# Mistra-UEA/Mistra

Hardware: AMD Instinct MI355X
Metric: chemistry-timesteps/sec (tot mechanism) (higher is better)
Workload: dtype f64; 1 GPU; tot mechanism, 100000 synthetic cells per GPU (100000 total), INTEGRATE_t(0,10 s), Ros3 rtol 1e-3; perturbed captured BTZ96 cloud states; cells_per_gpu=100000, failed_cells=0, parallelism=cells sharded over 1 GPU(s), no data-path collective

## Files before the change

mistra_amd/csrc/ros3_kernel.hip:

```cpp
#include <hip/hip_runtime.h>

#include <cstdint>
#include <type_traits>

#include "kernel_args.hpp"
#include "ros3_kernel.hpp"
#include "ros_methods.hpp"
#include "wave_ops.hpp"

namespace mistra {

namespace {

constexpr uint16_t kPosDiag = 0x8000, kPosNone = 0xFFFF;
constexpr int kRingSlots = 8;

#ifndef MISTRA_STREAM_GSUM_BARRIER
#define MISTRA_STREAM_GSUM_BARRIER 1
#endif
#ifndef MISTRA_STREAM_GSUM_CHAIN
#define MISTRA_STREAM_GSUM_CHAIN 1
#endif
#ifndef MISTRA_STREAM_SWEEP_BARRIER
#define MISTRA_STREAM_SWEEP_BARRIER 1
// ... 558 lines not shown
  const int n = __builtin_amdgcn_readfirstlane(P.nslots);
  gptr<u32x4> rp = G_(reinterpret_cast<const u32x4*>(P.recs)) + ((size_t)wave * (size_t)P.wave_slots * 64 + lane);
  asm volatile("s_waitcnt vmcnt(0)" : : : "memory");
  vm_ring_load<LOW, 0>(rp);       vm_ring_load<LOW, 1>(rp + 64);  vm_ring_load<LOW, 2>(rp + 128); vm_ring_load<LOW, 3>(rp + 192);
  vm_ring_load<LOW, 4>(rp + 256); vm_ring_load<LOW, 5>(rp + 320); vm_ring_load<LOW, 6>(rp + 384); vm_ring_load<LOW, 7>(rp + 448);
  rp += kRingSlots * 64;
  constexpr bool TRIM = MISTRA_STREAM_SCALE_TRIM && !LOW;
  const int n_refilled = TRIM ? n - kRingSlots : n;
#define MISTRA_SCALE_GROUP(K, REFILL)                                                \
    {                                                                                \
      const u32x4 a0 = vm_ring_take<LOW, K, REFILL ? 7 : 7 - K>();     if constexpr (REFILL) vm_ring_load<LOW, K>(rp + K * 64);         \
      const u32x4 a1 = vm_ring_take<LOW, K + 1, REFILL ? 7 : 6 - K>(); if constexpr (REFILL) vm_ring_load<LOW, K + 1>(rp + (K + 1) * 64); \
      const u32x4 a2 = vm_ring_take<LOW, K + 2, REFILL ? 7 : 5 - K>(); if constexpr (REFILL) vm_ring_load<LOW, K + 2>(rp + (K + 2) * 64); \
      const u32x4 a3 = vm_ring_take<LOW, K + 3, REFILL ? 7 : 4 - K>(); if constexpr (REFILL) vm_ring_load<LOW, K + 3>(rp + (K + 3) * 64); \
      const double v0 = lds_ld(a0.x), f0 = lds_ld(a0.y), v1 = lds_ld(a0.z), f1 = lds_ld(a0.w); \
      const double v2 = lds_ld(a1.x), f2 = lds_ld(a1.y), v3 = lds_ld(a1.z), f3 = lds_ld(a1.w); \
      const double v4 = lds_ld(a2.x), f4 = lds_ld(a2.y), v5 = lds_ld(a2.z), f5 = lds_ld(a2.w); \
      const double v6 = lds_ld(a3.x), f6 = lds_ld(a3.y), v7 = lds_ld(a3.z), f7 = lds_ld(a3.w); \
      lds_st(a0.x, v0 * f0); lds_st(a0.z, v1 * f1); lds_st(a1.x, v2 * f2); lds_st(a1.z, v3 * f3); \
      lds_st(a2.x, v4 * f4); lds_st(a2.z, v5 * f5); lds_st(a3.x, v6 * f6); lds_st(a3.z, v7 * f7); \
    }
  for (int i = 0; i < n_refilled; i += kRingSlots) {
    MISTRA_SCALE_GROUP(0, true) MISTRA_SCALE_GROUP(4, true)
    rp += kRingSlots * 64;
  }
  if constexpr (TRIM) {
    if (n > 0) { MISTRA_SCALE_GROUP(0, false) MISTRA_SCALE_GROUP(4, false) }
  }
#undef MISTRA_SCALE_GROUP
  asm volatile("s_waitcnt vmcnt(0)" : : : "memory");
}

#ifdef MISTRA_DIAG_STAMPS
__device__ unsigned long long g_dense_stamps[16];
#define MISTRA_STAMP(var) const unsigned long long var = clock64();
#define MISTRA_STAMP_ADD(slot, expr) if (threadIdx.x == 0) atomicAdd(&g_dense_stamps[slot], (unsigned long long)(expr));
#else
#define MISTRA_STAMP(var)
#define MISTRA_STAMP_ADD(slot, expr)
#endif
typedef double f64x4 __attribute__((ext_vector_type(4)));
typedef uint32_t u32x2 __attribute__((ext_vector_type(2)));
typedef __attribute__((address_space(3))) f64x4 lds_f64x4;
__device__ __forceinline__ f64x4 lds_ld4(uint32_t addr) { return *(const lds_f64x4*)(uintptr_t)addr; }
__device__ __forceinline__ void lds_st4(uint32_t addr, f64x4 v) { *(lds_f64x4*)(uintptr_t)addr = v; }
typedef __attribute__((address_space(3))) __attribute__((aligned(16))) f64x4 lds_f64x4_a16;
__device__ __forceinline__ f64x4 lds_ld4_a16(uint32_t addr) { return *(const lds_f64x4_a16*)(uintptr_t)addr; }
__device__ __forceinline__ void lds_st4_a16(uint32_t addr, f64x4 v) { *(lds_f64x4_a16*)(uintptr_t)addr = v; }

__device__ __forceinline__ uint32_t dense_slot(const u32x4 info, const uint32_t c, const uint32_t zero) {
  const uint64_t absent = (uint64_t)info.y | ((uint64_t)info.z << 32);
  const uint32_t idx = info.x + c - (uint32_t)__builtin_popcountll(absent & ((1ull << c) - 1ull));
  return ((absent >> c) & 1ull) ? zero : 8u * idx;
}
typedef __attribute__((address_space(3))) u32x4 lds_u32x4;
__device__ __forceinline__ u32x4 lds_ldu4(uint32_t addr) { return *(const lds_u32x4*)(uintptr_t)addr; }

__device__ __forceinline__ bool dense_is_storer(const int wave) { return wave == 1 || wave == 2 || wave == 3 || wave == 5; }
template <class MT, int NT>
__device__ __forceinline__ void dense_store_panel(const int P, const int wave, const int lane) {
  constexpr uint32_t NNZ = MT::NNZ, NVAR = MT::NVAR, H = NVAR - 64, ZERO = 8u * (NNZ + NVAR);
  constexpr uint32_t PB = 8u * (uint32_t)LdsLayout<MT, NT>::PANEL, BC = PB + 8192u, INFO = 8u * (uint32_t)LdsLayout<MT, NT>::DINFO;
  const uint32_t PL = PB + (uint32_t)(P & 1) * 4096u, PU = PL + 2048u;
  const int J0P = 4 * P, khalf = (wave == 3 || wave == 5) ? 2 : 0;
  const f64x4 rcp = lds_ld4(BC + 1024u + 32u * (uint32_t)(P & 1));
  if (wave & 1) {
    if (wave != 5) {
// ... 72 lines not shown
    a[2] = a[2] * rcp[2];
    a[3] = __builtin_fma(-a[2], d23, a[3]);
    a[3] = a[3] * rcp[3];
    b[1] = __builtin_fma(-l10, b[0], b[1]); b[2] = __builtin_fma(-l20, b[0], b[2]); b[3] = __builtin_fma(-l30, b[0], b[3]);
    b[2] = __builtin_fma(-l21, b[1], b[2]); b[3] = __builtin_fma(-l31, b[1], b[3]);
    b[3] = __builtin_fma(-l32, b[2], b[3]);
    lds_st4(PL + 32u * lane, a);
    lds_st4(PU + 32u * lane, b);
    if (lane == 0) lds_st4(BC + 1024u + 32u * (uint32_t)(P & 1), rcp);
  } else if (dense_is_storer(wave) && P > 0) {
    dense_store_panel<MT, NT>(P - 1, wave, lane);
  }
  MISTRA_STAMP(tc)
  lds_barrier();
  MISTRA_STAMP(td)
  if (I >= K2) {
    const double aop = (int)(16u * I + lcol) >= J0P + 4 ? -lds_ld(PL + 8u * ((16u * I + lcol) * 4u + lrow)) : 0.0;
    if (J0 >= K2) {
      const double bop = (int)(16u * J0 + lcol) >= J0P + 4 ? lds_ld(PU + 8u * ((16u * J0 + lcol) * 4u + lrow)) : 0.0;
      T0 = __builtin_amdgcn_mfma_f64_16x16x4f64(aop, bop, T0, 0, 0, 0);
    }
    if (J0 + 1 >= K2) {
      const double bop = (int)(16u * (J0 + 1) + lcol) >= J0P + 4 ? lds_ld(PU + 8u * ((16u * (J0 + 1) + lcol) * 4u + lrow)) : 0.0;
      T1 = __builtin_amdgcn_mfma_f64_16x16x4f64(aop, bop, T1, 0, 0, 0);
    }
  }
  MISTRA_STAMP(te)
#ifdef MISTRA_DIAG_STAMPS
  acc[0] += tb - ta; acc[1] += tc - tb; acc[2] += td - tc; acc[3] += te - td; acc[4] += 1;
#endif
}

#define MISTRA_FIN_F(J, C) "v_fmac_f64_dpp %[x" #C "], -%[x" #C "], %[l] row_newbcast:" #J " row_mask:0xf bank_mask:0xf\n\t"
#define MISTRA_FIN_FROM_15(J) MISTRA_FIN_F(J, 15)
#define MISTRA_FIN_FROM_14(J) MISTRA_FIN_F(J, 14) MISTRA_FIN_FROM_15(J)
#define MISTRA_FIN_FROM_13(J) MISTRA_FIN_F(J, 13) MISTRA_FIN_FROM_14(J)
#define MISTRA_FIN_FROM_12(J) MISTRA_FIN_F(J, 12) MISTRA_FIN_FROM_13(J)
#define MISTRA_FIN_FROM_11(J) MISTRA_FIN_F(J, 11) MISTRA_FIN_FROM_12(J)
#define MISTRA_FIN_FROM_10(J) MISTRA_FIN_F(J, 10) MISTRA_FIN_FROM_11(J)
#define MISTRA_FIN_FROM_9(J) MISTRA_FIN_F(J, 9) MISTRA_FIN_FROM_10(J)
#define MISTRA_FIN_FROM_8(J) MISTRA_FIN_F(J, 8) MISTRA_FIN_FROM_9(J)
#define MISTRA_FIN_FROM_7(J) MISTRA_FIN_F(J, 7) MISTRA_FIN_FROM_8(J)
#define MISTRA_FIN_FROM_6(J) MISTRA_FIN_F(J, 6) MISTRA_FIN_FROM_7(J)
#define MISTRA_FIN_FROM_5(J) MISTRA_FIN_F(J, 5) MISTRA_FIN_FROM_6(J)
#define MISTRA_FIN_FROM_4(J) MISTRA_FIN_F(J, 4) MISTRA_FIN_FROM_5(J)
#define MISTRA_FIN_FROM_3(J) MISTRA_FIN_F(J, 3) MISTRA_FIN_FROM_4(J)
#define MISTRA_FIN_FROM_2(J) MISTRA_FIN_F(J, 2) MISTRA_FIN_FROM_3(J)
#define MISTRA_FIN_FROM_1(J) MISTRA_FIN_F(J, 1) MISTRA_FIN_FROM_2(J)
#define MISTRA_FIN_XS [x0] "+v"(x0), [x1] "+v"(x1), [x2] "+v"(x2), [x3] "+v"(x3), [x4] "+v"(x4), [x5] "+v"(x5), [x6] "+v"(x6), [x7] "+v"(x7), \
                      [x8] "+v"(x8), [x9] "+v"(x9), [x10] "+v"(x10), [x11] "+v"(x11), [x12] "+v"(x12), [x13] "+v"(x13), [x14] "+v"(x14), [x15] "+v"(x15)
#define MISTRA_FIN_PIVOT(J, J1)                                                                                                       \
  {                                                                                                                                   \
    double dg, l;                                                                                                                     \
    asm volatile("s_nop 1\n\tv_mov_b64_dpp %[dg], %[x] row_newbcast:" #J " row_mask:0xf bank_mask:0xf" : [dg] "=v"(dg) : [x] "v"(x##J));       \
    const double R = 1.0 / dg;                                                                                                        \
    constexpr uint32_t GE = ((0xffffu << J) & 0xffffu) * 0x10001u, GT = ((0xffffu << J1) & 0xffffu) * 0x10001u;                       \
    asm volatile("v_mov_b64 %[l], %[nz]\n\t"                                                                                          \
                 "s_mov_b32 exec_lo, %[gt]\n\ts_mov_b32 exec_hi, %[gt]\n\t"                                                           \
                 "v_mul_f64 %[l], %[x" #J "], %[R]\n\t"                                                                               \
                 "v_mul_f64 %[x" #J "], %[x" #J "], %[R]\n\t"                                                                         \
                 "s_mov_b32 exec_lo, %[ge]\n\ts_mov_b32 exec_hi, %[ge]\n\t"                                                           \
                 MISTRA_FIN_FROM_##J1(J)                                                                                              \
                 "s_mov_b64 exec, -1"                                                                                                 \
                 : [l] "=&v"(l), MISTRA_FIN_XS : [R] "v"(R), [nz] "v"(nz), [gt] "i"((int)GT), [ge] "i"((int)GE));                               \
  }
template <class MT, int NT>
__device__ __attribute__((noinline)) void dense_finish(const f64x4 T, const int lane) {
  constexpr uint32_t NNZ = MT::NNZ, NVAR = MT::NVAR, H = NVAR - 64, ZERO = 8u * (NNZ + NVAR);
  constexpr uint32_t INFO = 8u * (uint32_t)LdsLayout<MT, NT>::DINFO, RDIAG = 8u * (NNZ + NVAR + 4u);
  constexpr uint32_t BUF = 8u * (uint32_t)LdsLayout<MT, NT>::PANEL, STRIDE = 144u;
  const uint32_t lrow = (uint32_t)(lane >> 4), i = (uint32_t)(lane & 15);
  MISTRA_STAMP(tf0)
#pragma unroll
  for (int r = 0; r < 4; r++) lds_st(BUF + STRIDE * (lrow + 4u * r) + 8u * i, T[r]);
  const f64x4 q0 = lds_ld4_a16(BUF + STRIDE * i), q1 = lds_ld4_a16(BUF + STRIDE * i + 32u), q2 = lds_ld4_a16(BUF + STRIDE * i + 64u), q3 = lds_ld4_a16(BUF + STRIDE * i + 96u);
  double x0 = q0[0], x1 = q0[1], x2 = q0[2], x3 = q0[3], x4 = q1[0], x5 = q1[1], x6 = q1[2], x7 = q1[3];
  double x8 = q2[0], x9 = q2[1], x10 = q2[2], x11 = q2[3], x12 = q3[0], x13 = q3[1], x14 = q3[2], x15 = q3[3];
  const u32x4 info = lds_ldu4(INFO + 16u * (48u + i));
  const uint32_t cb = 16u + 4u * lrow;
  uint32_t idx = info.x + 32u + cb - (uint32_t)__builtin_popcount(info.y) - (uint32_t)__builtin_popcount(info.z & ((1u << cb) - 1u));
  uint32_t at[4];
#pragma unroll
  for (int k = 0; k < 4; k++) {
    const uint32_t absent = (info.z >> (cb + (uint32_t)k)) & 1u;
    at[k] = absent ? ZERO : 8u * idx;
    idx += 1u - absent;
  }
  const double nz = -0.0;
  MISTRA_FIN_PIVOT(0, 1) MISTRA_FIN_PIVOT(1, 2) MISTRA_FIN_PIVOT(2, 3) MISTRA_FIN_PIVOT(3, 4) MISTRA_FIN_PIVOT(4, 5)
  MISTRA_FIN_PIVOT(5, 6) MISTRA_FIN_PIVOT(6, 7) MISTRA_FIN_PIVOT(7, 8) MISTRA_FIN_PIVOT(8, 9) MISTRA_FIN_PIVOT(9, 10)
  MISTRA_FIN_PIVOT(10, 11) MISTRA_FIN_PIVOT(11, 12) MISTRA_FIN_PIVOT(12, 13) MISTRA_FIN_PIVOT(13, 14) MISTRA_FIN_PIVOT(14, 15)
  MISTRA_STAMP(tf1)
  lds_st4_a16(BUF + STRIDE * i, f64x4{x0, x1, x2, x3}); lds_st4_a16(BUF + STRIDE * i + 32u, f64x4{x4, x5, x6, x7});
  lds_st4_a16(BUF + STRIDE * i + 64u, f64x4{x8, x9, x10, x11}); lds_st4_a16(BUF + STRIDE * i + 96u, f64x4{x12, x13, x14, x15});
  const f64x4 v = lds_ld4_a16(BUF + STRIDE * i + 32u * lrow);
  const double R = 1.0 / lds_ld(BUF + STRIDE * i + 8u * i);
#pragma unroll
  for (int k = 0; k < 4; k++) {
    const uint32_t c = 4u * lrow + (uint32_t)k;
    if (at[k] != ZERO) lds_st(at[k], c > i ? v[k] * R : v[k]);
  }
  if (lrow == 0) lds_st(RDIAG + 8u * (H + 48u + i), R);
  MISTRA_STAMP(tf2)
#ifdef MISTRA_DIAG_STAMPS
  if ((lane & 63) == 0) { atomicAdd(&g_dense_stamps[13], tf1 - tf0); atomicAdd(&g_dense_stamps[14], tf2 - tf1); }
#endif
}
#undef MISTRA_FIN_PIVOT
#undef MISTRA_FIN_XS
#undef MISTRA_FIN_F
#undef MISTRA_FIN_FROM_1
#undef MISTRA_FIN_FROM_2
#undef MISTRA_FIN_FROM_3
#undef MISTRA_FIN_FROM_4
#undef MISTRA_FIN_FROM_5
#undef MISTRA_FIN_FROM_6
#undef MISTRA_FIN_FROM_7
#undef MISTRA_FIN_FROM_8
#undef MISTRA_FIN_FROM_9
#undef MISTRA_FIN_FROM_10
#undef MISTRA_FIN_FROM_11
#undef MISTRA_FIN_FROM_12
#undef MISTRA_FIN_FROM_13
#undef MISTRA_FIN_FROM_14
#undef MISTRA_FIN_FROM_15

template <class MT, int NT>
__device__ __attribute__((noinline)) f64x4 dense_lu(int lane) {
  static_assert(NT == 512 && MT::DENSE_ND == 64, "eight waves, two 16x16 tiles each");
  constexpr int KB = MT::DENSE_KB;
  constexpr uint32_t NNZ = MT::NNZ, NVAR = MT::NVAR, H = NVAR - 64, JM = H - 4 * KB, ZERO = 8u * (NNZ + NVAR);
  constexpr uint32_t INFO = 8u * (uint32_t)LdsLayout<MT, NT>::DINFO, RDIAG = 8u * (NNZ + NVAR + 4u);
  const int wave = __builtin_amdgcn_readfirstlane((int)(threadIdx.x >> 6));
  const uint32_t I = (uint32_t)(wave >> 1), J0 = 2u * (uint32_t)(wave & 1), lrow = (uint32_t)(lane >> 4), lcol = (uint32_t)(lane & 15);
  MISTRA_STAMP(t0)
  f64x4 T0, T1;
#pragma unroll
  for (int r = 0; r < 4; r++) {
    const u32x4 info = lds_ldu4(INFO + 16u * (16u * I + lrow + 4u * r));
    T0[r] = lds_ld(dense_slot(info, 16u * J0 + lcol, ZERO));
    T1[r] = lds_ld(dense_slot(info, 16u * J0 + 16u + lcol, ZERO));
  }
  constexpr uint32_t SCH = 8u * (uint32_t)LdsLayout<MT, NT>::SCHUR;
  typedef __attribute__((address_space(3))) uint16_t lds_u16;
  const uint32_t wtab = SCH + 2u * ((uint32_t)I * KB * 64u + (uint32_t)lane);
  const uint32_t utab = SCH + 2u * (4u * KB * 64u + (uint32_t)(wave & 1) * KB * 128u + (uint32_t)lane);
  uint32_t wslot[KB];
  double wl[KB];
  static_assert(KB % 2 == 0, "two batches of Schur steps");
#pragma unroll
  for (int half = 0; half < 2; half++) {
    constexpr int HB = KB / 2;
    uint32_t us0[HB], us1[HB];
#pragma unroll
    for (int kk = 0; kk < HB; kk++) {
      const int k = half * HB + kk;
      wslot[k] = 8u * (uint32_t)*(const lds_u16*)(uintptr_t)(wtab + 128u * k);
      us0[kk] = 8u * (uint32_t)*(const lds_u16*)(uintptr_t)(utab + 256u * k);
// ... 10 lines not shown
    __builtin_amdgcn_sched_barrier(0);
#pragma unroll
    for (int kk = 0; kk < HB; kk++) {
      T0 = __builtin_amdgcn_mfma_f64_16x16x4f64(-wl[half * HB + kk], u0[kk], T0, 0, 0, 0);
      T1 = __builtin_amdgcn_mfma_f64_16x16x4f64(-wl[half * HB + kk], u1[kk], T1, 0, 0, 0);
    }
  }
  double rj[KB / 2];
#pragma unroll
  for (int k2 = 0; k2 < KB / 2; k2++) rj[k2] = lds_ld(RDIAG + 8u * (JM + 4u * (2u * k2 + (uint32_t)(wave & 1)) + lrow));
  MISTRA_STAMP(t1)
  lds_barrier();
  {
    static_assert(KB % 2 == 0, "the two waves of a block row take every other Schur step");
    if (wave & 1) {
#pragma unroll
      for (int k = 1; k < KB; k += 2)
        if (wslot[k] != ZERO) lds_st(wslot[k], wl[k] * rj[k / 2]);
    } else {
#pragma unroll
      for (int k = 0; k < KB; k += 2)
        if (wslot[k] != ZERO) lds_st(wslot[k], wl[k] * rj[k / 2]);
    }
  }
  MISTRA_STAMP(t2)
  MISTRA_STAMP_ADD(0, t1 - t0) MISTRA_STAMP_ADD(1, t2 - t1) MISTRA_STAMP_ADD(9, 1)
#ifndef MISTRA_DENSE_UNROLL
#define MISTRA_DENSE_UNROLL 12
#endif
#ifndef MISTRA_DIAG_DENSE_PANELS
#define MISTRA_DIAG_DENSE_PANELS 12
#endif
  static_assert(MISTRA_DIAG_DENSE_PANELS <= 12, "the panels end where the in-wave finish begins");
#ifdef MISTRA_DIAG_STAMPS
  unsigned long long acc[5] = {0, 0, 0, 0, 0};
  MISTRA_STAMP(tp0)
#pragma unroll 1
  for (int P = 0; P < MISTRA_DIAG_DENSE_PANELS; P++) dense_panel<MT, NT>(T0, T1, P, wave, lane, acc);
  MISTRA_STAMP(tp1)
  MISTRA_STAMP_ADD(2, acc[0]) MISTRA_STAMP_ADD(3, acc[1]) MISTRA_STAMP_ADD(4, acc[2]) MISTRA_STAMP_ADD(5, acc[3]) MISTRA_STAMP_ADD(8, acc[4]) MISTRA_STAMP_ADD(12, tp1 - tp0)
#else
#pragma unroll MISTRA_DENSE_UNROLL
  for (int P = 0; P < MISTRA_DIAG_DENSE_PANELS; P++) dense_panel<MT, NT>(T0, T1, P, wave, lane);
#endif
  if (dense_is_storer(wave)) dense_store_panel<MT, NT>(11, wave, lane);
#ifdef MISTRA_DIAG_STAMPS
  lds_barrier();
  MISTRA_STAMP(tz)
  MISTRA_STAMP_ADD(11, tz - t0)
#endif
  return T1;
}

}

template <class MT, int NT, int VARIANT, int METHOD = kRos3>
__global__ __launch_bounds__(NT, MT::WAVES_PER_SIMD) void ros3_integrate_kernel(const KernelArgs a) {
  constexpr bool PROF = VARIANT == 1, DUMP = VARIANT == 2, TRACE = VARIANT == 4, SERIES = VARIANT == 5, FLUX = VARIANT == 6, DENSE = VARIANT == 7, OPT = VARIANT == 3 || TRACE || SERIES || FLUX || DENSE;
  constexpr bool OPS = VARIANT == 8;
  static_assert(!OPS || METHOD == kRos3, "the operators are Ros3 instantiations (ros_unit_kernel.hip): no method is involved");
  static_assert(!TRACE || METHOD == kRos3, "the step-control trace is a Ros3 instantiation (ros_unit_kernel.hip)");
  static_assert(METHOD == kRos3 || (OPT && METHOD >= kRos2 && METHOD <= kRodas4), "the method kernels are options instantiations");
  constexpr double kGamma1 = METHOD == kRos3 ? kRosGamma1 : kRosMethod<METHOD>.Gamma[0];
  constexpr int NVAR = MT::NVAR, NFIX = MT::NFIX, NREACT = MT::NREACT, NNZ = MT::NNZ, NCONST = MT::NCONST;
  constexpr int NW = NT / 64;
  constexpr int SPT = (NVAR + NT - 1) / NT, RPT = (NREACT + NT - 1) / NT;
  constexpr int JPT = (MT::NJNZ + NT - 1) / NT, ZPT = (NNZ - MT::NJNZ + NT - 1) / NT;
  using L = LdsLayout<MT, NT>;

  extern __shared__ __attribute__((aligned(16))) double lds[];
  double* const M = lds + L::M;
  double* const XS = M + NNZ;
  double* const X = lds + L::X;
  double* const AB = lds + L::AB;
  double* const JBp = lds + L::JB;
  double* const red = lds + L::RED;
  int* const flags = reinterpret_cast<int*>(lds + L::FLAGS);

// ... 1091 lines not shown
    }
    if constexpr (SERIES) {
      if (++leg >= a.nleg) break;
    }
  } while (SERIES);
}

#ifndef MISTRA_METHOD_TU
template <class MT, int NT>
hipError_t launch_ros3(const KernelArgs& a, hipStream_t stream, bool* lds_configured) {
  constexpr size_t lds_bytes = LdsLayout<MT, NT>::TOTAL * sizeof(double);
  bool& configured = *lds_configured;
  auto kern = ros3_integrate_kernel<MT, NT, 0>;
  auto kern_prof = ros3_integrate_kernel<MT, NT, 1>;
  auto kern_dump = ros3_integrate_kernel<MT, NT, 2>;
  auto kern_opt = ros3_integrate_kernel<MT, NT, 3>;
  if (!configured) {
    for (const void* k : {reinterpret_cast<const void*>(kern), reinterpret_cast<const void*>(kern_prof), reinterpret_cast<const void*>(kern_dump),
                          reinterpret_cast<const void*>(kern_opt)}) {
      hipError_t e = hipFuncSetAttribute(k, hipFuncAttributeMaxDynamicSharedMemorySize, (int)lds_bytes);
      if (e != hipSuccess) return e;
    }
    configured = true;
  }
  if (a.ncell <= 0) return hipSuccess;
  if (a.dump) hipLaunchKernelGGL(kern_dump, dim3((unsigned)a.ncell), dim3(NT), lds_bytes, stream, a);
  else if (a.prof) hipLaunchKernelGGL(kern_prof, dim3((unsigned)a.ncell), dim3(NT), lds_bytes, stream, a);
  else if (a.opt) hipLaunchKernelGGL(kern_opt, dim3((unsigned)a.ncell), dim3(NT), lds_bytes, stream, a);
  else hipLaunchKernelGGL(kern, dim3((unsigned)a.ncell), dim3(NT), lds_bytes, stream, a);
  return hipGetLastError();
}

#ifdef MISTRA_DIAG_STAMPS
extern "C" int mistra_diag_dense_stamps(unsigned long long* out16, int reset) {
  if (hipMemcpyFromSymbol(out16, HIP_SYMBOL(g_dense_stamps), 16 * sizeof(unsigned long long)) != hipSuccess) return 1;
  if (reset) {
    unsigned long long z[16] = {0};
    if (hipMemcpyToSymbol(HIP_SYMBOL(g_dense_stamps), z, sizeof z) != hipSuccess) return 1;
  }
  return 0;
}
#endif

template hipError_t launch_ros3<GasTraits, kGasNT>(const KernelArgs&, hipStream_t, bool*);
template hipError_t launch_ros3<AerTraits, kAerNT>(const KernelArgs&, hipStream_t, bool*);
template hipError_t launch_ros3<TotTraits, kTotNT>(const KernelArgs&, hipStream_t, bool*);
#endif

}
```

mistra_amd/csrc/ros3_kernel.hpp:

```cpp
#pragma once
#include <hip/hip_runtime.h>

#include "kernel_args.hpp"

namespace mistra {

#ifndef MISTRA_GAS_NT
#define MISTRA_GAS_NT 64
#endif
#ifndef MISTRA_AER_NT
#define MISTRA_AER_NT 256
#endif
#ifndef MISTRA_TOT_NT
#define MISTRA_TOT_NT 512
#endif
#ifndef MISTRA_GAS_WPS
#define MISTRA_GAS_WPS 3
#endif
#ifndef MISTRA_AER_WPS
#define MISTRA_AER_WPS 2
#endif
#ifndef MISTRA_AER_SCALE_PASS
#define MISTRA_AER_SCALE_PASS 1
#endif
#ifndef MISTRA_TOT_DENSE
#define MISTRA_TOT_DENSE 1
#endif
#ifndef MISTRA_TOT_WPS
#define MISTRA_TOT_WPS 2
#endif
constexpr int kGasNT = MISTRA_GAS_NT, kAerNT = MISTRA_AER_NT, kTotNT = MISTRA_TOT_NT;

struct GasTraits { static constexpr int NVAR = 102, NFIX = 3, NREACT = 331, NNZ = 1110, NB = 568, NCONST = 2, NJNZ = 945, TAIL_REGS = 1, MAX_TEMPS = 10, WAVES_PER_SIMD = MISTRA_GAS_WPS, DENSE_ND = 0, DENSE_KB = 0; static constexpr bool RING_LOW = true, SCALE_PASS = false, RCT_LDS = false; };
struct AerTraits { static constexpr int NVAR = 257, NFIX = 5, NREACT = 979, NNZ = 6579, NB = 1598, NCONST = 2, NJNZ = 2831, TAIL_REGS = 2, MAX_TEMPS = 192, WAVES_PER_SIMD = MISTRA_AER_WPS, DENSE_ND = 0, DENSE_KB = 0; static constexpr bool RING_LOW = false, SCALE_PASS = MISTRA_AER_SCALE_PASS, RCT_LDS = true; };
struct TotTraits { static constexpr int NVAR = 417, NFIX = 7, NREACT = 1627, NNZ = 13503, NB = 2628, NCONST = 2, NJNZ = 4709, TAIL_REGS = 2, MAX_TEMPS = 768, WAVES_PER_SIMD = MISTRA_TOT_WPS, DENSE_ND = MISTRA_TOT_DENSE ? 64 : 0, DENSE_KB = MISTRA_TOT_DENSE ? 14 : 0; static constexpr bool RING_LOW = false, SCALE_PASS = true, RCT_LDS = false; };
constexpr int kResidentMaxWps = 2;

constexpr int round_up2(int x) { return (x + 1) & ~1; }
constexpr int spare_cells(int nt) { return nt >= 128 ? 64 : 32; }
constexpr int max_i(int a, int b) { return a > b ? a : b; }

template <class MT, int NT>
struct LdsLayout {
  static constexpr int M = 0;
  static constexpr int X = M + round_up2(MT::NNZ + 2 * MT::NVAR + 4 + MT::MAX_TEMPS);
  static constexpr int AB = X + round_up2(MT::NVAR + MT::NFIX + MT::NCONST);
  static constexpr int AB_TRASH = max_i(MT::NREACT, MT::NB);
  static constexpr int JVS_CELLS = (MT::NJNZ + NT - 1) / NT * NT;
  static constexpr int SPARE = spare_cells(NT);
  static constexpr bool MERGE_FUN_JAC = JVS_CELLS + round_up2(AB_TRASH + SPARE) <= MT::NNZ;
  static constexpr int JB = MERGE_FUN_JAC ? M + JVS_CELLS : AB;
  static constexpr int A_CELLS = MERGE_FUN_JAC ? MT::NREACT : AB_TRASH;
  static constexpr bool RCT_IN_LDS = MERGE_FUN_JAC && MT::RCT_LDS;
  static constexpr int RCT = AB + round_up2(A_CELLS + SPARE);
  static constexpr int RED = RCT + (RCT_IN_LDS ? round_up2(MT::NREACT) : 0);
  static constexpr int RED_H = NT == 64 ? 1 : 16, RED_HEXIT = NT == 64 ? 2 : 31, RED_CELLS = NT == 64 ? 4 : 32;
  static constexpr int FLAGS = RED + RED_CELLS;
  static constexpr int DINFO = FLAGS + 2;
  static constexpr int SCHUR = DINFO + (MT::DENSE_ND > 0 ? 64 * 2 : 0);
  static constexpr int SCHUR_WORDS = MT::DENSE_ND > 0 ? 8 * MT::DENSE_KB * 64 / 2 : 0;
  static constexpr int TOTAL = SCHUR + SCHUR_WORDS / 2;
  static constexpr int PANEL = AB;
  static constexpr int PANEL_CELLS = 2 * 2 * 64 * 4 + 2 * 64 + 4;
  static_assert(MT::DENSE_ND == 0 || PANEL_CELLS <= A_CELLS + SPARE, "panel buffers must fit the product array");
  static_assert(TOTAL * 8 <= 160 * 1024, "cell state does not fit the 160 KiB LDS of a gfx950 CU");
  static_assert(NT % 64 == 0 && NT <= 1024 && NT / 64 <= 32, "workgroup size");
};

template <class MT, int NT>
hipError_t launch_ros3(const KernelArgs& a, hipStream_t stream, bool* lds_configured);

template <class MT, int NT, int VARIANT, int METHOD>
hipError_t launch_ros_unit(const KernelArgs& a, hipStream_t stream, bool* lds_configured);

}
```

Baseline: 27930 chemistry-timesteps/s.

## Replace dense LU panel sweep with blocked 16x16 tile factorization using MFMA Schur updates

The dense 64x64 trailing block of the tot-mechanism LU is factored by default (tile-from 0) with a blocked right-looking scheme instead of the column-panel loop. Each step factors a 16x16 diagonal tile in one wave with DPP row broadcasts. L and U tiles are solved in parallel by two other waves, and every wave then applies an MFMA 16x16x4 Schur update to its trailing tiles. The aim is to cut the number of serialized panel steps and barriers by using whole-tile MFMA updates. In exchange it adds extra LDS tile buffers, more LDS stores to scatter results back to sparse slots, and more barriers per block column.

```diff
diff --git a/mistra_amd/csrc/ros3_kernel.hip b/mistra_amd/csrc/ros3_kernel.hip
--- a/mistra_amd/csrc/ros3_kernel.hip
+++ b/mistra_amd/csrc/ros3_kernel.hip
@@ -614,7 +614,7 @@
 }
 
 #ifdef MISTRA_DIAG_STAMPS
-__device__ unsigned long long g_dense_stamps[16];
+__device__ unsigned long long g_dense_stamps[24];
 #define MISTRA_STAMP(var) const unsigned long long var = clock64();
 #define MISTRA_STAMP_ADD(slot, expr) if (threadIdx.x == 0) atomicAdd(&g_dense_stamps[slot], (unsigned long long)(expr));
 #else
@@ -753,21 +753,22 @@
 }
 
 #define MISTRA_FIN_F(J, C) "v_fmac_f64_dpp %[x" #C "], -%[x" #C "], %[l] row_newbcast:" #J " row_mask:0xf bank_mask:0xf\n\t"
-#define MISTRA_FIN_FROM_15(J) MISTRA_FIN_F(J, 15)
-#define MISTRA_FIN_FROM_14(J) MISTRA_FIN_F(J, 14) MISTRA_FIN_FROM_15(J)
-#define MISTRA_FIN_FROM_13(J) MISTRA_FIN_F(J, 13) MISTRA_FIN_FROM_14(J)
-#define MISTRA_FIN_FROM_12(J) MISTRA_FIN_F(J, 12) MISTRA_FIN_FROM_13(J)
-#define MISTRA_FIN_FROM_11(J) MISTRA_FIN_F(J, 11) MISTRA_FIN_FROM_12(J)
-#define MISTRA_FIN_FROM_10(J) MISTRA_FIN_F(J, 10) MISTRA_FIN_FROM_11(J)
-#define MISTRA_FIN_FROM_9(J) MISTRA_FIN_F(J, 9) MISTRA_FIN_FROM_10(J)
-#define MISTRA_FIN_FROM_8(J) MISTRA_FIN_F(J, 8) MISTRA_FIN_FROM_9(J)
-#define MISTRA_FIN_FROM_7(J) MISTRA_FIN_F(J, 7) MISTRA_FIN_FROM_8(J)
-#define MISTRA_FIN_FROM_6(J) MISTRA_FIN_F(J, 6) MISTRA_FIN_FROM_7(J)
-#define MISTRA_FIN_FROM_5(J) MISTRA_FIN_F(J, 5) MISTRA_FIN_FROM_6(J)
-#define MISTRA_FIN_FROM_4(J) MISTRA_FIN_F(J, 4) MISTRA_FIN_FROM_5(J)
-#define MISTRA_FIN_FROM_3(J) MISTRA_FIN_F(J, 3) MISTRA_FIN_FROM_4(J)
-#define MISTRA_FIN_FROM_2(J) MISTRA_FIN_F(J, 2) MISTRA_FIN_FROM_3(J)
-#define MISTRA_FIN_FROM_1(J) MISTRA_FIN_F(J, 1) MISTRA_FIN_FROM_2(J)
+#define MISTRA_DPP_FROM_15(F, J) F(J, 15)
+#define MISTRA_DPP_FROM_14(F, J) F(J, 14) MISTRA_DPP_FROM_15(F, J)
+#define MISTRA_DPP_FROM_13(F, J) F(J, 13) MISTRA_DPP_FROM_14(F, J)
+#define MISTRA_DPP_FROM_12(F, J) F(J, 12) MISTRA_DPP_FROM_13(F, J)
+#define MISTRA_DPP_FROM_11(F, J) F(J, 11) MISTRA_DPP_FROM_12(F, J)
+#define MISTRA_DPP_FROM_10(F, J) F(J, 10) MISTRA_DPP_FROM_11(F, J)
+#define MISTRA_DPP_FROM_9(F, J) F(J, 9) MISTRA_DPP_FROM_10(F, J)
+#define MISTRA_DPP_FROM_8(F, J) F(J, 8) MISTRA_DPP_FROM_9(F, J)
+#define MISTRA_DPP_FROM_7(F, J) F(J, 7) MISTRA_DPP_FROM_8(F, J)
+#define MISTRA_DPP_FROM_6(F, J) F(J, 6) MISTRA_DPP_FROM_7(F, J)
+#define MISTRA_DPP_FROM_5(F, J) F(J, 5) MISTRA_DPP_FROM_6(F, J)
+#define MISTRA_DPP_FROM_4(F, J) F(J, 4) MISTRA_DPP_FROM_5(F, J)
+#define MISTRA_DPP_FROM_3(F, J) F(J, 3) MISTRA_DPP_FROM_4(F, J)
+#define MISTRA_DPP_FROM_2(F, J) F(J, 2) MISTRA_DPP_FROM_3(F, J)
+#define MISTRA_DPP_FROM_1(F, J) F(J, 1) MISTRA_DPP_FROM_2(F, J)
+#define MISTRA_DPP_FROM_16(F, J)
 #define MISTRA_FIN_XS [x0] "+v"(x0), [x1] "+v"(x1), [x2] "+v"(x2), [x3] "+v"(x3), [x4] "+v"(x4), [x5] "+v"(x5), [x6] "+v"(x6), [x7] "+v"(x7), \
                       [x8] "+v"(x8), [x9] "+v"(x9), [x10] "+v"(x10), [x11] "+v"(x11), [x12] "+v"(x12), [x13] "+v"(x13), [x14] "+v"(x14), [x15] "+v"(x15)
 #define MISTRA_FIN_PIVOT(J, J1)                                                                                                       \
@@ -781,15 +782,15 @@
                  "v_mul_f64 %[l], %[x" #J "], %[R]\n\t"                                                                               \
                  "v_mul_f64 %[x" #J "], %[x" #J "], %[R]\n\t"                                                                         \
                  "s_mov_b32 exec_lo, %[ge]\n\ts_mov_b32 exec_hi, %[ge]\n\t"                                                           \
-                 MISTRA_FIN_FROM_##J1(J)                                                                                              \
+                 MISTRA_DPP_FROM_##J1(MISTRA_FIN_F, J)                                                                                             \
                  "s_mov_b64 exec, -1"                                                                                                 \
                  : [l] "=&v"(l), MISTRA_FIN_XS : [R] "v"(R), [nz] "v"(nz), [gt] "i"((int)GT), [ge] "i"((int)GE));                               \
   }
-template <class MT, int NT>
-__device__ __attribute__((noinline)) void dense_finish(const f64x4 T, const int lane) {
+template <class MT, int NT, bool LAST>
+__device__ __forceinline__ void dense_diag_tile(const f64x4 T, const int lane, const uint32_t BUF) {
   constexpr uint32_t NNZ = MT::NNZ, NVAR = MT::NVAR, H = NVAR - 64, ZERO = 8u * (NNZ + NVAR);
   constexpr uint32_t INFO = 8u * (uint32_t)LdsLayout<MT, NT>::DINFO, RDIAG = 8u * (NNZ + NVAR + 4u);
-  constexpr uint32_t BUF = 8u * (uint32_t)LdsLayout<MT, NT>::PANEL, STRIDE = 144u;
+  constexpr uint32_t STRIDE = 144u;
   const uint32_t lrow = (uint32_t)(lane >> 4), i = (uint32_t)(lane & 15);
   MISTRA_STAMP(tf0)
 #pragma unroll
@@ -797,15 +798,17 @@
   const f64x4 q0 = lds_ld4_a16(BUF + STRIDE * i), q1 = lds_ld4_a16(BUF + STRIDE * i + 32u), q2 = lds_ld4_a16(BUF + STRIDE * i + 64u), q3 = lds_ld4_a16(BUF + STRIDE * i + 96u);
   double x0 = q0[0], x1 = q0[1], x2 = q0[2], x3 = q0[3], x4 = q1[0], x5 = q1[1], x6 = q1[2], x7 = q1[3];
   double x8 = q2[0], x9 = q2[1], x10 = q2[2], x11 = q2[3], x12 = q3[0], x13 = q3[1], x14 = q3[2], x15 = q3[3];
-  const u32x4 info = lds_ldu4(INFO + 16u * (48u + i));
-  const uint32_t cb = 16u + 4u * lrow;
-  uint32_t idx = info.x + 32u + cb - (uint32_t)__builtin_popcount(info.y) - (uint32_t)__builtin_popcount(info.z & ((1u << cb) - 1u));
   uint32_t at[4];
-#pragma unroll
-  for (int k = 0; k < 4; k++) {
-    const uint32_t absent = (info.z >> (cb + (uint32_t)k)) & 1u;
-    at[k] = absent ? ZERO : 8u * idx;
-    idx += 1u - absent;
+  if constexpr (LAST) {
+    const u32x4 info = lds_ldu4(INFO + 16u * (48u + i));
+    const uint32_t cb = 16u + 4u * lrow;
+    uint32_t idx = info.x + 32u + cb - (uint32_t)__builtin_popcount(info.y) - (uint32_t)__builtin_popcount(info.z & ((1u << cb) - 1u));
+#pragma unroll
+    for (int k = 0; k < 4; k++) {
+      const uint32_t absent = (info.z >> (cb + (uint32_t)k)) & 1u;
+      at[k] = absent ? ZERO : 8u * idx;
+      idx += 1u - absent;
+    }
   }
   const double nz = -0.0;
   MISTRA_FIN_PIVOT(0, 1) MISTRA_FIN_PIVOT(1, 2) MISTRA_FIN_PIVOT(2, 3) MISTRA_FIN_PIVOT(3, 4) MISTRA_FIN_PIVOT(4, 5)
@@ -814,37 +817,138 @@
   MISTRA_STAMP(tf1)
   lds_st4_a16(BUF + STRIDE * i, f64x4{x0, x1, x2, x3}); lds_st4_a16(BUF + STRIDE * i + 32u, f64x4{x4, x5, x6, x7});
   lds_st4_a16(BUF + STRIDE * i + 64u, f64x4{x8, x9, x10, x11}); lds_st4_a16(BUF + STRIDE * i + 96u, f64x4{x12, x13, x14, x15});
-  const f64x4 v = lds_ld4_a16(BUF + STRIDE * i + 32u * lrow);
-  const double R = 1.0 / lds_ld(BUF + STRIDE * i + 8u * i);
-#pragma unroll
-  for (int k = 0; k < 4; k++) {
-    const uint32_t c = 4u * lrow + (uint32_t)k;
-    if (at[k] != ZERO) lds_st(at[k], c > i ? v[k] * R : v[k]);
-  }
-  if (lrow == 0) lds_st(RDIAG + 8u * (H + 48u + i), R);
+  if constexpr (LAST) {
+    const f64x4 v = lds_ld4_a16(BUF + STRIDE * i + 32u * lrow);
+    const double R = 1.0 / lds_ld(BUF + STRIDE * i + 8u * i);
+#pragma unroll
+    for (int k = 0; k < 4; k++) {
+      const uint32_t c = 4u * lrow + (uint32_t)k;
+      if (at[k] != ZERO) lds_st(at[k], c > i ? v[k] * R : v[k]);
+    }
+    if (lrow == 0) lds_st(RDIAG + 8u * (H + 48u + i), R);
+  }
   MISTRA_STAMP(tf2)
 #ifdef MISTRA_DIAG_STAMPS
-  if ((lane & 63) == 0) { atomicAdd(&g_dense_stamps[13], tf1 - tf0); atomicAdd(&g_dense_stamps[14], tf2 - tf1); }
+  if ((lane & 63) == 0) { atomicAdd(&g_dense_stamps[LAST ? 13 : 16], tf1 - tf0); atomicAdd(&g_dense_stamps[LAST ? 14 : 17], tf2 - tf1); }
 #endif
 }
+template <class MT, int NT>
+__device__ __attribute__((noinline)) void dense_finish(const f64x4 T, const int lane) {
+  typedef LdsLayout<MT, NT> L;
+  constexpr uint32_t BUF = 8u * (uint32_t)(L::DENSE_TILES ? L::TILE_D + L::TILE_CELLS : L::PANEL);
+  dense_diag_tile<MT, NT, true>(T, lane, BUF);
+}
 #undef MISTRA_FIN_PIVOT
+#undef MISTRA_FIN_F
+
+struct DenseRow { double x0, x1, x2, x3, x4, x5, x6, x7, x8, x9, x10, x11, x12, x13, x14, x15; };
+__device__ __forceinline__ void dense_row_load(DenseRow& X, const uint32_t at) {
+  const f64x4 q0 = lds_ld4_a16(at), q1 = lds_ld4_a16(at + 32u), q2 = lds_ld4_a16(at + 64u), q3 = lds_ld4_a16(at + 96u);
+  X.x0 = q0[0]; X.x1 = q0[1]; X.x2 = q0[2]; X.x3 = q0[3]; X.x4 = q1[0]; X.x5 = q1[1]; X.x6 = q1[2]; X.x7 = q1[3];
+  X.x8 = q2[0]; X.x9 = q2[1]; X.x10 = q2[2]; X.x11 = q2[3]; X.x12 = q3[0]; X.x13 = q3[1]; X.x14 = q3[2]; X.x15 = q3[3];
+}
+__device__ __forceinline__ void dense_row_store(const DenseRow& X, const uint32_t at) {
+  lds_st4_a16(at, f64x4{X.x0, X.x1, X.x2, X.x3}); lds_st4_a16(at + 32u, f64x4{X.x4, X.x5, X.x6, X.x7});
+  lds_st4_a16(at + 64u, f64x4{X.x8, X.x9, X.x10, X.x11}); lds_st4_a16(at + 96u, f64x4{X.x12, X.x13, X.x14, X.x15});
+}
+#define MISTRA_TS_L(J, C) "v_fmac_f64_dpp %[x" #C "], -%[d" #C "], %[x" #J "] row_newbcast:" #J " row_mask:0xf bank_mask:0xf\n\t"
+#define MISTRA_TS_U(J, C) "v_fmac_f64_dpp %[x" #C "], -%[d" #J "], %[x" #J "] row_newbcast:" #C " row_mask:0xf bank_mask:0xf\n\t"
+#define MISTRA_TS_LP(J, J1) "v_mov_b64_dpp %[rj], %[R] row_newbcast:" #J " row_mask:0xf bank_mask:0xf\n\tv_mul_f64 %[x" #J "], %[x" #J "], %[rj]\n\t" MISTRA_DPP_FROM_##J1(MISTRA_TS_L, J)
+#define MISTRA_TS_UP(J, J1) MISTRA_DPP_FROM_##J1(MISTRA_TS_U, J)
+#define MISTRA_TS_ALL(P) P(0, 1) P(1, 2) P(2, 3) P(3, 4) P(4, 5) P(5, 6) P(6, 7) P(7, 8) P(8, 9) P(9, 10) P(10, 11) P(11, 12) P(12, 13) P(13, 14) P(14, 15) P(15, 16)
+#define MISTRA_TS_XS [x0] "+v"(X.x0), [x1] "+v"(X.x1), [x2] "+v"(X.x2), [x3] "+v"(X.x3), [x4] "+v"(X.x4), [x5] "+v"(X.x5), [x6] "+v"(X.x6), [x7] "+v"(X.x7), \
+                     [x8] "+v"(X.x8), [x9] "+v"(X.x9), [x10] "+v"(X.x10), [x11] "+v"(X.x11), [x12] "+v"(X.x12), [x13] "+v"(X.x13), [x14] "+v"(X.x14), [x15] "+v"(X.x15)
+#define MISTRA_TS_DS [d0] "v"(D.x0), [d1] "v"(D.x1), [d2] "v"(D.x2), [d3] "v"(D.x3), [d4] "v"(D.x4), [d5] "v"(D.x5), [d6] "v"(D.x6), [d7] "v"(D.x7), \
+                     [d8] "v"(D.x8), [d9] "v"(D.x9), [d10] "v"(D.x10), [d11] "v"(D.x11), [d12] "v"(D.x12), [d13] "v"(D.x13), [d14] "v"(D.x14), [d15] "v"(D.x15)
+template <bool LSIDE>
+__device__ __forceinline__ void dense_tile_solve(DenseRow& X, double& R, const uint32_t DB, const uint32_t XB, const int lane) {
+  const uint32_t i = (uint32_t)(lane & 15);
+  DenseRow D;
+  dense_row_load(D, DB + 144u * i);
+  dense_row_load(X, XB + 144u * i);
+  if constexpr (LSIDE) {
+    R = 1.0 / lds_ld(DB + 144u * i + 8u * i);
+    double rj;
+    asm volatile("s_nop 1\n\t" MISTRA_TS_ALL(MISTRA_TS_LP) : [rj] "=&v"(rj), MISTRA_TS_XS : [R] "v"(R), MISTRA_TS_DS);
+  } else {
+    asm volatile("s_nop 1\n\t" MISTRA_TS_ALL(MISTRA_TS_UP) : MISTRA_TS_XS : MISTRA_TS_DS);
+  }
+  dense_row_store(X, XB + 144u * i);
+  if constexpr (LSIDE)
+    if (lane < 16) lds_st(DB + 144u * i + 128u, R);
+}
+#undef MISTRA_TS_L
+#undef MISTRA_TS_U
+#undef MISTRA_TS_LP
+#undef MISTRA_TS_UP
+#undef MISTRA_TS_ALL
+#undef MISTRA_TS_XS
+#undef MISTRA_TS_DS
 #undef MISTRA_FIN_XS
-#undef MISTRA_FIN_F
-#undef MISTRA_FIN_FROM_1
-#undef MISTRA_FIN_FROM_2
-#undef MISTRA_FIN_FROM_3
-#undef MISTRA_FIN_FROM_4
-#undef MISTRA_FIN_FROM_5
-#undef MISTRA_FIN_FROM_6
-#undef MISTRA_FIN_FROM_7
-#undef MISTRA_FIN_FROM_8
-#undef MISTRA_FIN_FROM_9
-#undef MISTRA_FIN_FROM_10
-#undef MISTRA_FIN_FROM_11
-#undef MISTRA_FIN_FROM_12
-#undef MISTRA_FIN_FROM_13
-#undef MISTRA_FIN_FROM_14
-#undef MISTRA_FIN_FROM_15
+#undef MISTRA_DPP_FROM_1
+#undef MISTRA_DPP_FROM_2
+#undef MISTRA_DPP_FROM_3
+#undef MISTRA_DPP_FROM_4
+#undef MISTRA_DPP_FROM_5
+#undef MISTRA_DPP_FROM_6
+#undef MISTRA_DPP_FROM_7
+#undef MISTRA_DPP_FROM_8
+#undef MISTRA_DPP_FROM_9
+#undef MISTRA_DPP_FROM_10
+#undef MISTRA_DPP_FROM_11
+#undef MISTRA_DPP_FROM_12
+#undef MISTRA_DPP_FROM_13
+#undef MISTRA_DPP_FROM_14
+#undef MISTRA_DPP_FROM_15
+#undef MISTRA_DPP_FROM_16
+
+template <class MT, int NT>
+__device__ __forceinline__ void dense_tile_store_d(const int K, const uint32_t DB, const int lane) {
+  constexpr uint32_t NNZ = MT::NNZ, NVAR = MT::NVAR, H = NVAR - 64, TRASH = 8u * (NNZ + NVAR + 2u);
+  constexpr uint32_t INFO = 8u * (uint32_t)LdsLayout<MT, NT>::DINFO, RDIAG = 8u * (NNZ + NVAR + 4u);
+  const uint32_t q = (uint32_t)(lane >> 4), i = (uint32_t)(lane & 15), c0 = 16u * (uint32_t)K, cb = c0 + 4u * q;
+  const u32x4 info = lds_ldu4(INFO + 16u * (c0 + i));
+  const f64x4 v = lds_ld4_a16(DB + 144u * i + 32u * q);
+  const double R = 1.0 / lds_ld(DB + 144u * i + 8u * i);
+  const uint64_t absent = (uint64_t)info.y | ((uint64_t)info.z << 32);
+  uint32_t idx = info.x + cb - (uint32_t)__builtin_popcountll(absent & ((1ull << cb) - 1ull));
+  const uint32_t ab = (uint32_t)(absent >> cb);
+#pragma unroll
+  for (int k = 0; k < 4; k++) {
+    const uint32_t a = (ab >> k) & 1u, c = 4u * q + (uint32_t)k;
+    lds_st(a ? TRASH : 8u * idx, c > i ? v[k] * R : v[k]);
+    idx += 1u - a;
+  }
+  if (q == 0) lds_st(RDIAG + 8u * (H + c0 + i), R);
+}
+__device__ __forceinline__ void dense_row_to_slots(const DenseRow& X, const double f, const bool scaled, const uint32_t row, const uint32_t c0, const uint32_t INFO, const uint32_t TRASH) {
+  const u32x4 info = lds_ldu4(INFO + 16u * row);
+  const uint64_t absent = (uint64_t)info.y | ((uint64_t)info.z << 32);
+  uint32_t idx = info.x + c0 - (uint32_t)__builtin_popcountll(absent & ((1ull << c0) - 1ull));
+  const uint32_t ab = (uint32_t)(absent >> c0);
+#define MISTRA_TS_ST(k) { const uint32_t a = (ab >> k) & 1u; lds_st(a ? TRASH : 8u * idx, scaled ? X.x##k * f : X.x##k); idx += 1u - a; }
+  MISTRA_TS_ST(0) MISTRA_TS_ST(1) MISTRA_TS_ST(2) MISTRA_TS_ST(3) MISTRA_TS_ST(4) MISTRA_TS_ST(5) MISTRA_TS_ST(6) MISTRA_TS_ST(7)
+  MISTRA_TS_ST(8) MISTRA_TS_ST(9) MISTRA_TS_ST(10) MISTRA_TS_ST(11) MISTRA_TS_ST(12) MISTRA_TS_ST(13) MISTRA_TS_ST(14) MISTRA_TS_ST(15)
+#undef MISTRA_TS_ST
+}
+template <class MT, int NT>
+__device__ __forceinline__ void dense_tile_store_l(const DenseRow& X, const int K, const int lane) {
+  constexpr uint32_t NNZ = MT::NNZ, NVAR = MT::NVAR;
+  const int q = (lane >> 4) < 2 - K ? (lane >> 4) : 2 - K;
+  dense_row_to_slots(X, 0.0, false, 16u * (uint32_t)(K + 1 + q) + (uint32_t)(lane & 15), 16u * (uint32_t)K, 8u * (uint32_t)LdsLayout<MT, NT>::DINFO, 8u * (NNZ + NVAR + 2u));
+}
+template <class MT, int NT>
+__device__ __forceinline__ void dense_tile_store_u(const int K, const uint32_t DB, const uint32_t UB, const uint32_t TB, const int lane) {
+  constexpr uint32_t NNZ = MT::NNZ, NVAR = MT::NVAR;
+  const int q = (lane >> 4) < 2 - K ? (lane >> 4) : 2 - K;
+  const uint32_t i = (uint32_t)(lane & 15), at = UB + TB * (uint32_t)q + 8u * i;
+  DenseRow Y;
+  Y.x0 = lds_ld(at); Y.x1 = lds_ld(at + 144u); Y.x2 = lds_ld(at + 2u * 144u); Y.x3 = lds_ld(at + 3u * 144u);
+  Y.x4 = lds_ld(at + 4u * 144u); Y.x5 = lds_ld(at + 5u * 144u); Y.x6 = lds_ld(at + 6u * 144u); Y.x7 = lds_ld(at + 7u * 144u);
+  Y.x8 = lds_ld(at + 8u * 144u); Y.x9 = lds_ld(at + 9u * 144u); Y.x10 = lds_ld(at + 10u * 144u); Y.x11 = lds_ld(at + 11u * 144u);
+  Y.x12 = lds_ld(at + 12u * 144u); Y.x13 = lds_ld(at + 13u * 144u); Y.x14 = lds_ld(at + 14u * 144u); Y.x15 = lds_ld(at + 15u * 144u);
+  dense_row_to_slots(Y, lds_ld(DB + 144u * i + 128u), true, 16u * (uint32_t)K + i, 16u * (uint32_t)(K + 1 + q), 8u * (uint32_t)LdsLayout<MT, NT>::DINFO, 8u * (NNZ + NVAR + 2u));
+}
 
 template <class MT, int NT>
 __device__ __attribute__((noinline)) f64x4 dense_lu(int lane) {
@@ -921,18 +1025,108 @@
 #define MISTRA_DIAG_DENSE_PANELS 12
 #endif
   static_assert(MISTRA_DIAG_DENSE_PANELS <= 12, "the panels end where the in-wave finish begins");
+  constexpr int FROM = MISTRA_DENSE_TILE_FROM, NPANEL = MISTRA_DIAG_DENSE_PANELS < 4 * FROM ? MISTRA_DIAG_DENSE_PANELS : 4 * FROM;
 #ifdef MISTRA_DIAG_STAMPS
   unsigned long long acc[5] = {0, 0, 0, 0, 0};
   MISTRA_STAMP(tp0)
 #pragma unroll 1
-  for (int P = 0; P < MISTRA_DIAG_DENSE_PANELS; P++) dense_panel<MT, NT>(T0, T1, P, wave, lane, acc);
+  for (int P = 0; P < NPANEL; P++) dense_panel<MT, NT>(T0, T1, P, wave, lane, acc);
   MISTRA_STAMP(tp1)
   MISTRA_STAMP_ADD(2, acc[0]) MISTRA_STAMP_ADD(3, acc[1]) MISTRA_STAMP_ADD(4, acc[2]) MISTRA_STAMP_ADD(5, acc[3]) MISTRA_STAMP_ADD(8, acc[4]) MISTRA_STAMP_ADD(12, tp1 - tp0)
 #else
 #pragma unroll MISTRA_DENSE_UNROLL
-  for (int P = 0; P < MISTRA_DIAG_DENSE_PANELS; P++) dense_panel<MT, NT>(T0, T1, P, wave, lane);
+  for (int P = 0; P < NPANEL; P++) dense_panel<MT, NT>(T0, T1, P, wave, lane);
 #endif
-  if (dense_is_storer(wave)) dense_store_panel<MT, NT>(11, wave, lane);
+  if constexpr (FROM == 3) {
+    if (dense_is_storer(wave)) dense_store_panel<MT, NT>(11, wave, lane);
+  } else {
+    typedef LdsLayout<MT, NT> L;
+    constexpr uint32_t TB = 8u * (uint32_t)L::TILE_CELLS, DBUF = 8u * (uint32_t)L::TILE_D, LBUF = 8u * (uint32_t)L::TILE_L, UBUF = 8u * (uint32_t)L::TILE_U;
+    if constexpr (FROM > 0)
+      if (dense_is_storer(wave)) dense_store_panel<MT, NT>(4 * FROM - 1, wave, lane);
+#ifndef MISTRA_DENSE_TILE_UNROLL
+#define MISTRA_DENSE_TILE_UNROLL 3
+#endif
+#pragma unroll MISTRA_DENSE_TILE_UNROLL
+    for (int K = FROM; K < 3; K++) {
+      const int LS = K == 0 ? 1 : 4, US = K == 1 ? 1 : 6;
+      if (K > FROM || FROM > 0) lds_barrier();
+      {
+        const bool odd = K & 1;
+        const f64x4 TK = odd ? T1 : T0;
+        if ((int)I > K && (wave & 1) == (K >> 1)) {
+          const uint32_t at = LBUF + TB * (I - 1u) + 8u * lcol;
+#pragma unroll
+          for (int r = 0; r < 4; r++) lds_st(at + 144u * (lrow + 4u * r), TK[r]);
+        }
+        if ((int)I == K) {
+          if ((int)J0 > K) {
+            const uint32_t at = UBUF + TB * (J0 - 1u) + 144u * lcol + 8u * lrow;
+#pragma unroll
+            for (int r = 0; r < 4; r++) lds_st(at + 32u * r, T0[r]);
+          }
+          if ((int)J0 + 1 > K) {
+            const uint32_t at = UBUF + TB * J0 + 144u * lcol + 8u * lrow;
+#pragma unroll
+            for (int r = 0; r < 4; r++) lds_st(at + 32u * r, T1[r]);
+          }
+        }
+#ifdef MISTRA_DIAG_STAMPS
+        if (wave == 4 && lane == 0) atomicAdd(&g_dense_stamps[23], 1ull);
+#endif
+      }
+      {
+        DenseRow X;
+        double R;
+        const uint32_t DB = DBUF + TB * (uint32_t)(K & 1);
+        MISTRA_STAMP(tc0)
+        if (wave == 2 * K + (K >> 1)) dense_diag_tile<MT, NT, false>((K & 1) ? T1 : T0, lane, DB);
+        MISTRA_STAMP(tc1)
+        lds_barrier();
+        MISTRA_STAMP(tc2)
+        const uint32_t xt = TB * (uint32_t)(K + ((lane >> 4) < 2 - K ? (lane >> 4) : 2 - K));
+        if (wave == LS) dense_tile_solve<true>(X, R, DB, LBUF + xt, lane);
+        else if (wave == US) dense_tile_solve<false>(X, R, DB, UBUF + xt, lane);
+        else if (wave == 2 * K + (K >> 1)) dense_tile_store_d<MT, NT>(K, DB, lane);
+        MISTRA_STAMP(tc3)
+        lds_barrier();
+        MISTRA_STAMP(tc4)
+        if ((int)I > K) {
+          const uint32_t la = LBUF + TB * (I - 1u) + 144u * lcol + 8u * lrow;
+          const double a0 = -lds_ld(la), a1 = -lds_ld(la + 32u), a2 = -lds_ld(la + 64u), a3 = -lds_ld(la + 96u);
+          if ((int)J0 > K) {
+            const uint32_t ua = UBUF + TB * (J0 - 1u) + 144u * lcol + 8u * lrow;
+            const double b0 = lds_ld(ua), b1 = lds_ld(ua + 32u), b2 = lds_ld(ua + 64u), b3 = lds_ld(ua + 96u);
+            T0 = __builtin_amdgcn_mfma_f64_16x16x4f64(a0, b0, T0, 0, 0, 0);
+            T0 = __builtin_amdgcn_mfma_f64_16x16x4f64(a1, b1, T0, 0, 0, 0);
+            T0 = __builtin_amdgcn_mfma_f64_16x16x4f64(a2, b2, T0, 0, 0, 0);
+            T0 = __builtin_amdgcn_mfma_f64_16x16x4f64(a3, b3, T0, 0, 0, 0);
+          }
+          if ((int)J0 + 1 > K) {
+            const uint32_t ua = UBUF + TB * J0 + 144u * lcol + 8u * lrow;
+            const double b0 = lds_ld(ua), b1 = lds_ld(ua + 32u), b2 = lds_ld(ua + 64u), b3 = lds_ld(ua + 96u);
+            T1 = __builtin_amdgcn_mfma_f64_16x16x4f64(a0, b0, T1, 0, 0, 0);
+            T1 = __builtin_amdgcn_mfma_f64_16x16x4f64(a1, b1, T1, 0, 0, 0);
+            T1 = __builtin_amdgcn_mfma_f64_16x16x4f64(a2, b2, T1, 0, 0, 0);
+            T1 = __builtin_amdgcn_mfma_f64_16x16x4f64(a3, b3, T1, 0, 0, 0);
+          }
+        }
+        MISTRA_STAMP(tc5)
+#ifdef MISTRA_DIAG_STAMPS
+        if (wave == 2 * K + (K >> 1) && lane == 0) atomicAdd(&g_dense_stamps[18], tc2 - tc1);
+        if (wave == LS && lane == 0) { atomicAdd(&g_dense_stamps[19], tc3 - tc2); atomicAdd(&g_dense_stamps[20], tc4 - tc3); }
+        if (wave == 7 && lane == 0) atomicAdd(&g_dense_stamps[21], tc5 - tc4);
+#endif
+        MISTRA_STAMP(tq0)
+        if (wave == LS) dense_tile_store_l<MT, NT>(X, K, lane);
+        else if (wave == US) dense_tile_store_u<MT, NT>(K, DB, UBUF + TB * (uint32_t)K, TB, lane);
+        MISTRA_STAMP(tq1)
+#ifdef MISTRA_DIAG_STAMPS
+        if (wave == LS && lane == 0) atomicAdd(&g_dense_stamps[22], tq1 - tq0);
+#endif
+      }
+    }
+  }
 #ifdef MISTRA_DIAG_STAMPS
   lds_barrier();
   MISTRA_STAMP(tz)
@@ -2090,10 +2284,10 @@
 }
 
 #ifdef MISTRA_DIAG_STAMPS
-extern "C" int mistra_diag_dense_stamps(unsigned long long* out16, int reset) {
-  if (hipMemcpyFromSymbol(out16, HIP_SYMBOL(g_dense_stamps), 16 * sizeof(unsigned long long)) != hipSuccess) return 1;
+extern "C" int mistra_diag_dense_stamps(unsigned long long* out24, int reset) {
+  if (hipMemcpyFromSymbol(out24, HIP_SYMBOL(g_dense_stamps), 24 * sizeof(unsigned long long)) != hipSuccess) return 1;
   if (reset) {
-    unsigned long long z[16] = {0};
+    unsigned long long z[24] = {0};
     if (hipMemcpyToSymbol(HIP_SYMBOL(g_dense_stamps), z, sizeof z) != hipSuccess) return 1;
   }
   return 0;
diff --git a/mistra_amd/csrc/ros3_kernel.hpp b/mistra_amd/csrc/ros3_kernel.hpp
--- a/mistra_amd/csrc/ros3_kernel.hpp
+++ b/mistra_amd/csrc/ros3_kernel.hpp
@@ -29,6 +29,10 @@
 #ifndef MISTRA_TOT_WPS
 #define MISTRA_TOT_WPS 2
 #endif
+#ifndef MISTRA_DENSE_TILE_FROM
+#define MISTRA_DENSE_TILE_FROM 0
+#endif
+static_assert(MISTRA_DENSE_TILE_FROM >= 0 && MISTRA_DENSE_TILE_FROM <= 3, "block columns 0 .. 2 have a tile step; 3 = none");
 constexpr int kGasNT = MISTRA_GAS_NT, kAerNT = MISTRA_AER_NT, kTotNT = MISTRA_TOT_NT;
 
 struct GasTraits { static constexpr int NVAR = 102, NFIX = 3, NREACT = 331, NNZ = 1110, NB = 568, NCONST = 2, NJNZ = 945, TAIL_REGS = 1, MAX_TEMPS = 10, WAVES_PER_SIMD = MISTRA_GAS_WPS, DENSE_ND = 0, DENSE_KB = 0; static constexpr bool RING_LOW = true, SCALE_PASS = false, RCT_LDS = false; };
@@ -59,10 +63,17 @@
   static constexpr int DINFO = FLAGS + 2;
   static constexpr int SCHUR = DINFO + (MT::DENSE_ND > 0 ? 64 * 2 : 0);
   static constexpr int SCHUR_WORDS = MT::DENSE_ND > 0 ? 8 * MT::DENSE_KB * 64 / 2 : 0;
-  static constexpr int TOTAL = SCHUR + SCHUR_WORDS / 2;
+  static constexpr bool DENSE_TILES = MT::DENSE_ND > 0 && MISTRA_DENSE_TILE_FROM < 3;
+  static constexpr int TILE_STRIDE = 18, TILE_CELLS = 16 * TILE_STRIDE;
+  static constexpr int TILE_U = SCHUR + SCHUR_WORDS / 2;
+  static constexpr int TOTAL = TILE_U + (DENSE_TILES ? 3 * TILE_CELLS : 0);
   static constexpr int PANEL = AB;
   static constexpr int PANEL_CELLS = 2 * 2 * 64 * 4 + 2 * 64 + 4;
   static_assert(MT::DENSE_ND == 0 || PANEL_CELLS <= A_CELLS + SPARE, "panel buffers must fit the product array");
+  static constexpr int TILE_D = AB;
+  static constexpr int TILE_L = TILE_D + 2 * TILE_CELLS;
+  static_assert(!DENSE_TILES || 5 * TILE_CELLS <= A_CELLS + SPARE, "tile buffers must fit the product array");
+  static_assert((TOTAL + 2 * (NT / 64)) * 8 <= 160 * 1024, "cell state and the trace kernel's cells behind it do not fit the 160 KiB LDS of a gfx950 CU");
   static_assert(TOTAL * 8 <= 160 * 1024, "cell state does not fit the 160 KiB LDS of a gfx950 CU");
   static_assert(NT % 64 == 0 && NT <= 1024 && NT / 64 <= 32, "workgroup size");
 };
```

Measured after the change: 28740 chemistry-timesteps/s (median of 6 runs). 1.03x the previous value.
